# rvp-group/Splat-LOAM

Hardware: AMD Instinct MI355X
Metric: fwd+bwd Msplats/s (higher is better)
Workload: dtype f32; 1 GPU; 500000 surfels, 64x2048 spherical, 1 keyframe/GPU per iteration drawn from a window of 8 keyframes as Mapper.optimize does (sample_geometric, p=0.4): render fwd + mapper loss + bwd + fused Adam (one native sls_mapping_step per iteration); step=one bench step = 10 mapping iterations (1013 steps = 10130 timed iterations), N=500000, H=64, W=2048, keyframes=8, parallelism=keyframe-dp1, status_read=lagged-1, gradient_sums=float atomics

## Files before the change

splat_loam_amd/csrc/sls_sort.hip:

```cpp
#include <cstdlib>
#include "sls_common.hpp"
#include "sls_resort.hpp"
#include "sls_launch.hpp"

namespace sls {

#ifndef SLS_SORT_ROUNDS
#define SLS_SORT_ROUNDS 16
#endif
#ifndef SLS_SORT_WAVES
#define SLS_SORT_WAVES 8
#endif
constexpr int kSortRounds = SLS_SORT_ROUNDS;
constexpr int kSortWaveItems = kWave * kSortRounds;
constexpr int kSortMaxBins = 2048;
constexpr int kDepthKeyBits = 29;

__device__ __forceinline__ uint32_t load_count(const uint32_t *count_ptr, uint32_t cap)
{
    const uint32_t c = *count_ptr;
    return c < cap ? c : cap;
}

__device__ __forceinline__ void resort_verify(int nwin, const uint64_t *__restrict__ edges, uint32_t *__restrict__ flag);
// ... 390 lines not shown

template <typename KeyT, int BITS>
static int tile_sort_emit_chunks(const KeyT *kin, const uint32_t *vin, KeyT *kout, uint32_t *vout,
                                 const uint32_t *chunk_start, uint32_t cap, int shift, uint32_t *cnt, uint32_t *totals,
                                 int nchunks, uint2 *ranges_out, int nranges, uint32_t packed_val_mask, hipStream_t st,
                                 const BlockMaskArgs &bm)
{
    {
        ScopedTimer tm(T_SORT_ROWSCAN, st);
        hipLaunchKernelGGL(sort_rowscan_kernel, dim3(1 << BITS), dim3(256), 0, st, cnt, (const uint32_t *)nullptr, cap, nchunks,
                           totals, nchunks);
    }
    SLS_LAUNCH_CHECK("sort_rowscan_kernel");
    {
        ScopedTimer tm(T_SORT_SCATTER, st);
        const int nblocks = (nchunks + SortBlock<BITS>::kWaves - 1) / SortBlock<BITS>::kWaves;
        hipLaunchKernelGGL((sort_scatter_chunks_kernel<KeyT, BITS>), dim3(nblocks), dim3(64 * SortBlock<BITS>::kWaves), 0, st,
                           kin, vin, kout, vout, chunk_start, cap, shift, (const uint32_t *)cnt, (const uint32_t *)totals,
                           nchunks, ranges_out, nranges, packed_val_mask, bm);
    }
    SLS_LAUNCH_CHECK("sort_scatter_chunks_kernel");
    return SLS_OK;
}

static size_t sort_core_bytes(uint64_t cap)
{
    const uint64_t nchunks = (cap + kSortWaveItems - 1) / kSortWaveItems;
    return (size_t)(kSortMaxBins * (nchunks ? nchunks : 1) + kSortMaxBins) * sizeof(uint32_t);
}
size_t sort_scratch_bytes(uint64_t cap)
{
    return sort_core_bytes(cap) + 2 * sizeof(uint64_t) * (size_t)cap + 64;
}
uint2 *sort_bmask_buffer(void *scratch, uint64_t cap)
{
    return (uint2 *)((char *)scratch + ((sort_core_bytes(cap) + 15) & ~(size_t)15));
}
uint64_t *sort_wide_buffer(void *scratch, uint64_t cap)
{
    return (uint64_t *)(sort_bmask_buffer(scratch, cap) + cap);
}

static void sort_plan(int nbits, int &npasses, int &bits)
{
    npasses = (nbits + 10) / 11;
    bits = (nbits + npasses - 1) / npasses;
    if (bits < 8) bits = 8;
}
int sort_passes(int nbits)
{
    int np, b;
    sort_plan(nbits, np, b);
    return np;
}

template <typename KeyT, int BITS>
static int radix_pass(const KeyT *kin, const uint32_t *vin, KeyT *kout, uint32_t *vout, const uint32_t *count_ptr,
                      uint32_t cap, int shift, uint32_t *cnt, uint32_t *totals, int nchunks, int ,
                      uint2 *ranges_out, int nranges, uint32_t packed_val_mask, hipStream_t st,
                      const BlockMaskArgs &bm)
{
    const int nblocks = (nchunks + SortBlock<BITS>::kWaves - 1) / SortBlock<BITS>::kWaves;
    {
        ScopedTimer tm(T_SORT_HIST, st);
        hipLaunchKernelGGL((sort_hist_kernel<KeyT, BITS>), dim3(nblocks), dim3(64 * SortBlock<BITS>::kWaves), 0, st, kin,
                           count_ptr, cap, shift, cnt, nchunks);
    }
    SLS_LAUNCH_CHECK("sort_hist_kernel");
    {
        ScopedTimer tm(T_SORT_ROWSCAN, st);
        hipLaunchKernelGGL(sort_rowscan_kernel, dim3(1 << BITS), dim3(256), 0, st, cnt, count_ptr, cap, nchunks, totals, 0);
    }
    SLS_LAUNCH_CHECK("sort_rowscan_kernel");
    {
        ScopedTimer tm(T_SORT_SCATTER, st);
        hipLaunchKernelGGL((sort_scatter_kernel<KeyT, BITS>), dim3(nblocks), dim3(64 * SortBlock<BITS>::kWaves), 0, st, kin, vin, kout, vout,
                           count_ptr, cap, shift, (const uint32_t *)cnt, (const uint32_t *)totals, nchunks, ranges_out,
                           nranges, packed_val_mask, bm);
    }
    SLS_LAUNCH_CHECK("sort_scatter_kernel");
    return SLS_OK;
}

template <typename KeyT>
static int radix_sort_pairs_t(KeyT *keys, uint32_t *vals, KeyT *keys_tmp, uint32_t *vals_tmp,
                              const uint32_t *count_ptr, uint32_t cap, int nbits, void *scratch,
                              size_t scratch_bytes, int *result_in_tmp, hipStream_t st,
                              uint2 *ranges_out = nullptr, int nranges = 0, bool drop_sorted_keys = false,
                              int base_shift = 0, BlockMaskArgs bm = BlockMaskArgs{ nullptr, 1, 1.0f, 1 })
{
    *result_in_tmp = 0;
    if (cap == 0 || nbits <= 0) return SLS_OK;
    if (scratch_bytes < sort_scratch_bytes(cap)) {
        set_error("sort scratch too small: %zu < %zu", scratch_bytes, sort_scratch_bytes(cap));
        return SLS_E_SCRATCH;
    }
    const int nchunks = (int)(((uint64_t)cap + kSortWaveItems - 1) / kSortWaveItems);
    uint32_t *cnt = (uint32_t *)scratch;
    int npasses, bits;
    sort_plan(nbits, npasses, bits);
    if (ranges_out && npasses != 1) {
        set_error("internal: ranges need a single-pass sort");
        return SLS_E_ARG;
    }
    uint32_t *totals = cnt + ((size_t)1 << bits) * nchunks;
    KeyT *kb[2] = { keys, keys_tmp };
    uint32_t *vb[2] = { vals, vals_tmp };
    for (int p = 0; p < npasses; ++p) {
        const int shift = base_shift + bits * p;
        const int src = p & 1, dst = src ^ 1;
        const uint32_t packed_val_mask = (vals == nullptr && base_shift > 0) ? ((1u << base_shift) - 1u) : 0u;
        int rc;
        KeyT *kout = (drop_sorted_keys && p + 1 == npasses) ? nullptr : kb[dst];
#define SLS_PASS(B) radix_pass<KeyT, B>(kb[src], vb[src], kout, vb[dst], count_ptr, cap, shift, cnt, totals, nchunks, \
                                        0, ranges_out, nranges, packed_val_mask, st,                           \
                                        (npasses == 1 ? bm : BlockMaskArgs{ nullptr, 1, 1.0f, 1 }))
        switch (bits) {
        case 8: rc = SLS_PASS(8); break;
        case 9: rc = SLS_PASS(9); break;
        case 10: rc = SLS_PASS(10); break;
        default: rc = SLS_PASS(11); break;
        }
#undef SLS_PASS
        if (rc) return rc;
    }
    *result_in_tmp = npasses & 1;
    return SLS_OK;
}

int radix_sort_pairs_u32(uint32_t *keys, uint32_t *vals, uint32_t *keys_tmp, uint32_t *vals_tmp,
                         const uint32_t *count_ptr, uint32_t cap, int nbits, void *scratch, size_t scratch_bytes,
                         int *result_in_tmp, hipStream_t st)
{
    return radix_sort_pairs_t<uint32_t>(keys, vals, keys_tmp, vals_tmp, count_ptr, cap, nbits, scratch,
                                        scratch_bytes, result_in_tmp, st);
}

int radix_sort_pairs_u64(uint64_t *keys, uint32_t *vals, uint64_t *keys_tmp, uint32_t *vals_tmp,
                         const uint32_t *count_ptr, uint32_t cap, int nbits, void *scratch, size_t scratch_bytes,
                         int *result_in_tmp, hipStream_t st)
{
    return radix_sort_pairs_t<uint64_t>(keys, vals, keys_tmp, vals_tmp, count_ptr, cap, nbits, scratch,
                                        scratch_bytes, result_in_tmp, st);
}

__global__ __launch_bounds__(kResortThreads) void resort_sort_kernel(int N, const uint32_t *__restrict__ prev_order,
                                                                     const uint32_t *__restrict__ keys_by_surfel,
                                                                     uint64_t *__restrict__ comp)
{
    __shared__ __attribute__((aligned(16))) ulonglong2 s_pairs[kResortThreads];
    resort_sort_window((int)blockIdx.x, N, prev_order, [&](uint32_t g) { return keys_by_surfel[g]; }, comp, s_pairs);
}

template <bool DIRECT, bool PRE>
__global__ __launch_bounds__(kResortThreads) void resort_merge_kernel(int N, const uint64_t *__restrict__ comp,
                                                                      uint32_t *__restrict__ order,
                                                                      uint64_t *__restrict__ edges,
                                                                      const uint32_t *__restrict__ tiles,
                                                                      uint32_t *__restrict__ block_sums, int GX,
                                                                      const uint2 *__restrict__ erec_box, DirectBin db,
                                                                      uint64_t *comp_out)
{
    static_assert(kResortWindow == 1024 && kResortThreads == 512, "a 256-block of positions = two waves of pairs");
    __shared__ __attribute__((aligned(16))) ulonglong2 s_pairs[kResortThreads];
    __shared__ uint32_t s_part[4][2];
    __shared__ uint32_t s_hist[DIRECT ? kDirectMaxBins : 1];
    __shared__ int s_diff[DIRECT ? kDirectMaxBins + 64 : 1];
    __shared__ int s_wide;
    __shared__ uint64_t s_win[PRE ? 2 * kResortWindow : 1];
    const bool use_diff = DIRECT && GX % 64 == 0 && db.bins % GX == 0 && db.bins / GX <= 64;
    if (DIRECT) {
        for (int d = threadIdx.x; d < db.bins; d += kResortThreads) s_hist[d] = 0u;
        for (int d = threadIdx.x; d < kDirectMaxBins + 64; d += kResortThreads) s_diff[d] = 0;
        if (threadIdx.x == 0) s_wide = 0;
    }
    const int base = blockIdx.x * kResortWindow - kResortWindow / 2, o0 = 2 * (int)threadIdx.x;
    uint64_t e[2];
    if (PRE) {
        uint64_t f[2][2];
#pragma unroll
        for (int a = 0; a < 2; ++a) {
            const int abase = ((int)blockIdx.x - 1 + a) * kResortWindow;
#pragma unroll
            for (int q = 0; q < 2; ++q) {
                const int pos = abase + bitonic_src(o0 + q);
                const uint64_t c = comp[min(max(pos, 0), N - 1)];
                f[a][q] = pos < 0 ? 0ull : (pos < N ? c : ~0ull);
            }
        }
#pragma unroll
        for (int a = 0; a < 2; ++a) {
            bitonic_pairs<kResortWindow>(f[a][0], f[a][1], s_pairs);
            s_win[a * kResortWindow + o0] = f[a][0];
            s_win[a * kResortWindow + o0 + 1] = f[a][1];
        }
        __syncthreads();
#pragma unroll
        for (int q = 0; q < 2; ++q) {
            const int o = bitonic_src(o0 + q);
            e[q] = o < kResortWindow / 2 ? s_win[kResortWindow / 2 + o] : s_win[kResortWindow + o - kResortWindow / 2];
        }
    } else {
#pragma unroll
        for (int q = 0; q < 2; ++q) {
            const int pos = base + bitonic_src(o0 + q);
            const uint64_t c = comp[min(max(pos, 0), N - 1)];
            e[q] = pos < 0 ? 0ull : (pos < N ? c : ~0ull);
        }
    }
    bitonic_pairs<kResortWindow>(e[0], e[1], s_pairs);
    if (comp_out) {
#pragma unroll
        for (int q = 0; q < 2; ++q) {
            const int pos = base + o0 + q;
            if (pos >= 0 && pos < N) comp_out[pos] = e[q];
        }
    }
    uint32_t v = 0;
    if (DIRECT) {
        uint2 er[2];
#pragma unroll
        for (int q = 0; q < 2; ++q) {
            const int pos = base + o0 + q;
            const bool real = pos >= 0 && pos < N;
            const uint32_t g = real ? (uint32_t)e[q] : 0u;
            er[q] = erec_box[g];
            if (!real) er[q].x = 0u;
            if (real) order[pos] = g;
        }
#pragma unroll
        for (int q = 0; q < 2; ++q) {
            const int pos = base + o0 + q;
            if (pos >= 0 && pos < N) db.serec[pos] = er[q];
            if (use_diff) count_rect_rows_diff(er[q].x, GX, s_hist, s_diff, &s_wide);
            else count_rect_tiles_wave(er[q].x, GX, s_hist);
        }
    } else {
#pragma unroll
        for (int q = 0; q < 2; ++q) {
            const int pos = base + o0 + q;
            const bool real = pos >= 0 && pos < N;
            const uint32_t g = real ? (uint32_t)e[q] : 0u;
            const uint32_t tv = tiles[g];
            v += real ? tv : 0u;
            if (real) order[pos] = g;
        }
#pragma unroll
        for (int off = 32; off > 0; off >>= 1) v += __shfl_down(v, off, 64);
        if ((threadIdx.x & 63) == 0) s_part[threadIdx.x >> 7][(threadIdx.x >> 6) & 1] = v;
    }
    const int lo = base < 0 ? -base : 0, hi = min(kResortWindow, N - base) - 1;
#pragma unroll
    for (int q = 0; q < 2; ++q) {
        if (o0 + q == lo) edges[2 * blockIdx.x + 0] = e[q];
        if (o0 + q == hi) edges[2 * blockIdx.x + 1] = e[q];
    }
    __syncthreads();
    if (DIRECT && use_diff && s_wide) {
        diff_finish(GX, db.bins, s_hist, s_diff, (int)threadIdx.x, kResortThreads);
        __syncthreads();
    }
    if (DIRECT) {
        for (int d = threadIdx.x; d < db.bins; d += kResortThreads) {
            const uint32_t c = s_hist[d];
            db.cnt[(size_t)d * db.stride + blockIdx.x] = c;
            if (db.coarse && c) atomicAdd(&db.coarse[(size_t)(blockIdx.x / kDirectGroup) * db.bins + d], c);
        }
    } else if (threadIdx.x < 4) {
        const int blk = (base + (int)threadIdx.x * 256) / 256;
        if (base + (int)threadIdx.x * 256 >= 0 && blk * 256 < N)
            block_sums[blk] = s_part[threadIdx.x][0] + s_part[threadIdx.x][1];
    }
}

__global__ __launch_bounds__(kDirectChunk) void gather_count_kernel(int N, int GX, const uint32_t *__restrict__ order,
                                                                    const uint2 *__restrict__ erec_box,
                                                                    const int4 *__restrict__ rect,
                                                                    const uint32_t *__restrict__ sbox, DirectBin db)
{
    __shared__ uint32_t s_hist[kDirectMaxBins];
    __shared__ int s_diff[kDirectMaxBins + 64];
    __shared__ int s_wide;
    const bool use_diff = GX % 64 == 0 && db.bins % GX == 0 && db.bins / GX <= 64;
    if ((int)threadIdx.x < db.bins) s_hist[threadIdx.x] = 0u;
    for (int d = threadIdx.x; d < kDirectMaxBins + 64; d += kDirectChunk) s_diff[d] = 0;
    if (threadIdx.x == 0) s_wide = 0;
    __syncthreads();
    const int pos = blockIdx.x * kDirectChunk + (int)threadIdx.x;
    uint2 er = make_uint2(0u, 0u);
    if (pos < N) {
        er = load_emit_record(erec_box, rect, sbox, order[pos]);
        if (db.serec) db.serec[pos] = er;
    }
    if (use_diff) count_rect_rows_diff(er.x, GX, s_hist, s_diff, &s_wide);
    else count_rect_tiles_wave(er.x, GX, s_hist);
    __syncthreads();
    if (use_diff && s_wide) {
        diff_finish(GX, db.bins, s_hist, s_diff, (int)threadIdx.x, kDirectChunk);
        __syncthreads();
    }
    if ((int)threadIdx.x < db.bins) {
        const uint32_t c = s_hist[threadIdx.x];
        db.cnt[(size_t)threadIdx.x * db.stride + blockIdx.x] = c;
        if (db.coarse && c) atomicAdd(&db.coarse[(size_t)(blockIdx.x / kDirectGroup) * db.bins + threadIdx.x], c);
    }
}

__device__ __forceinline__ void resort_verify(int nwin, const uint64_t *__restrict__ edges, uint32_t *__restrict__ flag)
{
    for (int b = threadIdx.x; b + 1 < nwin; b += 256)
        if (edges[2 * b + 1] >= edges[2 * (b + 1)]) atomicOr(flag, kResortFailed);
}

__device__ __forceinline__ uint32_t wave_max_scan(uint32_t v)
{
#define SLS_MAXDPP(ctrl_, rows_) v = max(v, (uint32_t)__builtin_amdgcn_update_dpp((int)v, (int)v, ctrl_, rows_, 0xF, false))
    SLS_MAXDPP(0x111, 0xF);
    SLS_MAXDPP(0x112, 0xF);
    SLS_MAXDPP(0x114, 0xF);
    SLS_MAXDPP(0x118, 0xF);
    SLS_MAXDPP(0x142, 0xA);
    SLS_MAXDPP(0x143, 0xC);
#undef SLS_MAXDPP
    return v;
}

constexpr uint32_t kHeavyWave = 1536;
constexpr int kHeavyParts = 4, kHeavyChunks = 16;
template <int BITS, bool PAIRS, int SPLIT>
__global__ __launch_bounds__(kDirectChunk / SPLIT) void bin_direct_kernel(int N, int GX, DirectBin db,
                                                                  const uint32_t *__restrict__ order,
                                                                  const uint2 *__restrict__ erec_box,
                                                                  const int4 *__restrict__ rect,
                                                                  const uint32_t *__restrict__ sbox, uint32_t cap,
                                                                  uint32_t *__restrict__ vals_out, BlockMaskArgs bm,
                                                                  uint2 *__restrict__ ranges_out, int nranges,
                                                                  uint32_t *__restrict__ total_out,
                                                                  uint32_t *__restrict__ overflow, int resort_windows,
                                                                  const uint64_t *__restrict__ resort_edges,
                                                                  uint32_t *__restrict__ fail_flag,
                                                                  uint32_t *__restrict__ status_mirror)
{
    constexpr int BINS = 1 << BITS, TPB = kDirectChunk / SPLIT, WAVES = TPB / 64;
    constexpr int PER = BINS > TPB ? BINS / TPB : 1;
    static_assert(BINS <= kDirectMaxBins && TPB % 64 == 0 && (BINS % TPB == 0 || BINS < TPB), "tiles dealt evenly to the threads");
    __shared__ uint32_t s_cur[WAVES * BINS];
    __shared__ uint32_t s_pre[BINS];
    __shared__ uint4 s_lane[WAVES][64];
    __shared__ uint32_t s_mark[WAVES][64];
    __shared__ uint32_t s_part[WAVES];
    __shared__ uint32_t s_ws[WAVES];
    const int tid = threadIdx.x, lane = tid & 63, w = tid >> 6;
    const int nhelp = SPLIT == 1 ? min(kHeavyChunks, db.nchunks) * (kHeavyParts - 1) : 0;
    const bool helper = (int)blockIdx.x < nhelp;
    const int chunk = helper ? (int)blockIdx.x / (kHeavyParts - 1) : ((int)blockIdx.x - nhelp) / SPLIT;
    const int sub = helper ? 0 : ((int)blockIdx.x - nhelp) % SPLIT;
    const int part = helper ? 1 + (int)blockIdx.x % (kHeavyParts - 1) : 0;
    const bool lead = !helper && chunk == 0 && sub == 0;
    if (resort_windows > 0 && lead) {
        for (int b = tid; b + 1 < resort_windows; b += TPB)
            if (resort_edges[2 * b + 1] >= resort_edges[2 * (b + 1)]) atomicOr(fail_flag, kResortFailed);
    }
    const int pos0 = db.pos0 + chunk * kDirectChunk;
    const int pos = pos0 + sub * TPB + tid;
    const bool real = pos >= 0 && pos < N;
    uint2 er = make_uint2(0u, 0u);
    uint32_t g = 0u;
    if (real) {
        g = order[pos];
// ... 359 lines not shown
        mask = (tile_mask && (uint32_t)(rc.y * rc.w) <= 64u) ? tile_mask[g] : ~0ull;
    }
    const uint64_t box_hi = wide ? ((uint64_t)sbox[g] << 32) : 0ull;
    const uint32_t nrect = (uint32_t)(rc.y * rc.w);
    if (nrect > 64u) mask = ~0ull;
    const uint32_t t = (i < N) ? (nrect <= 64u ? (uint32_t)__popcll(mask & (nrect >= 64u ? ~0ull : ((1ull << nrect) - 1ull))) : nrect) : 0u;
    uint32_t end;
    if (fused.block_sums) {
        __shared__ uint32_t s_wave[EW];
        __shared__ uint32_t s_pre[EW];
        if (fused.resort_windows > 0 && blockIdx.x == 0) resort_verify(fused.resort_windows, fused.resort_edges, fail_flag);
        const int lane = threadIdx.x & 63, wave = threadIdx.x >> 6;
        uint32_t pre = 0;
        for (int b = threadIdx.x; b < (int)blockIdx.x * (EB / 256); b += EB) pre += fused.block_sums[b];
#pragma unroll
        for (int off = 32; off > 0; off >>= 1) pre += __shfl_xor(pre, off, 64);
        uint32_t incl = t;
#pragma unroll
        for (int off = 1; off < 64; off <<= 1) {
            const uint32_t u = __shfl_up(incl, off, 64);
            if (lane >= off) incl += u;
        }
        if (lane == 63) s_wave[wave] = incl;
        if (lane == 0) s_pre[wave] = pre;
        __syncthreads();
        uint32_t wave_prefix = 0;
        for (int w = 0; w < wave; ++w) wave_prefix += s_wave[w];
        uint32_t block_prefix = 0;
#pragma unroll
        for (int w = 0; w < EW; ++w) block_prefix += s_pre[w];
        end = block_prefix + wave_prefix + incl;
        if (blockIdx.x == gridDim.x - 1 && threadIdx.x == EB - 1) *total_out = end;
    } else {
        end = (i < N) ? offsets[i] : 0u;
    }
    if (chunk_start && threadIdx.x == 0) {
        chunk_start[blockIdx.x] = end - t;
        if (blockIdx.x == gridDim.x - 1 && !fused.block_sums) chunk_start[gridDim.x] = offsets[N - 1];
    }
    if (chunk_start && fused.block_sums && blockIdx.x == gridDim.x - 1 && threadIdx.x == EB - 1) chunk_start[gridDim.x] = end;
    bool emit = i < N && t != 0u;
    uint32_t off = end - t;
    if (emit && end > cap) {
        if (overflow) atomicOr(overflow, 1u);
        if (off >= cap) emit = false;
    }
    if (emit) {
        uint32_t bit = 0;
        for (int y = 0; y < rc.w; ++y) {
            const uint32_t row = (uint32_t)(rc.z + y) * (uint32_t)GX;
            for (int k = 0; k < rc.y; ++k, ++bit) {
                if (bit < 64u && !((mask >> bit) & 1ull)) continue;
                int tx = rc.x + k;
                if (tx >= GX) tx -= GX;
                if (off < cap) {
                    const uint32_t tile = row + (uint32_t)tx;
                    if (wide) wide[off] = box_hi | (uint64_t)((tile << pack_shift) | g);
                    else if (vals) { tkeys[off] = tile; vals[off] = g; }
                    else tkeys[off] = (tile << pack_shift) | g;
                    if (hist_cnt) atomicAdd(&s_hist[tile], 1u);
                }
                ++off;
            }
        }
    }
    if (hist_cnt) {
        __syncthreads();
        for (int d = threadIdx.x; d < hist_bins; d += EB) hist_cnt[(size_t)d * gridDim.x + blockIdx.x] = s_hist[d];
    }
}

__global__ __launch_bounds__(256) void tile_ranges_kernel(const uint32_t *__restrict__ tkeys,
                                                          const uint32_t *__restrict__ vals,
                                                          const uint32_t *__restrict__ count_ptr, uint32_t cap,
                                                          const float *__restrict__ depth, uint2 *__restrict__ ranges,
                                                          uint64_t *__restrict__ keys64)
{
    const uint32_t R = load_count(count_ptr, cap);
    const uint32_t j = blockIdx.x * 256 + threadIdx.x;
    if (j >= R) return;
    const uint32_t t = tkeys[j];
    if (j == 0 || tkeys[j - 1] != t) ranges[t].x = j;
    if (j + 1 == R || tkeys[j + 1] != t) ranges[t].y = j + 1;
    if (keys64) keys64[j] = ((uint64_t)t << 32) | (uint64_t)__float_as_uint(depth[vals[j]]);
}

static int bits_for(uint32_t max_value)
{
    int b = 0;
    while (b < 32 && (max_value >> b) != 0) ++b;
    return b;
}

size_t order_scratch_bytes(int N)
{
    const size_t n = (size_t)(N > 0 ? N : 1);
    return sizeof(uint32_t) * (3 * n + (n + 255) / 256 + 64) + sort_scratch_bytes(n) + 16 + n / 32 + 128;
}

struct OrderScratch {
    uint32_t *keys, *keys_tmp, *vals_tmp, *block_sums, *n_dev;
    void *sort_scratch;
    uint64_t *comp;
    bool odd;
    OrderScratch(int N, void *scratch)
    {
        keys = (uint32_t *)scratch; keys_tmp = keys + N; vals_tmp = keys_tmp + N;
        block_sums = vals_tmp + N + 2;
        n_dev = block_sums + (N + 255) / 256;
        sort_scratch = (void *)(n_dev + 32);
        comp = (uint64_t *)(((uintptr_t)keys_tmp + 7) & ~(uintptr_t)7);
        odd = (sort_passes(kDepthKeyBits) & 1) != 0;
    }
};

void depth_order_key_buffers(int N, void *scratch, uint32_t *order, uint32_t **keys, uint32_t **vals0, uint32_t **n_dev)
{
    const OrderScratch s(N, scratch);
    *keys = s.keys;
    *vals0 = s.odd ? s.vals_tmp : order;
    *n_dev = s.n_dev;
}

uint64_t *resort_comp_buffer(int N, void *scratch) { return OrderScratch(N, scratch).comp; }

int launch_depth_order_scan(const DepthOrderScan &a, hipStream_t st, ScanHandoff *handoff)
{
    const int N = a.N, reuse_order = a.reuse_order;
    uint32_t *order = a.order;
    const DirectBin *direct = a.direct;
    if (a.scratch_bytes < order_scratch_bytes(N)) {
        set_error("depth-order scratch too small: %zu < %zu", a.scratch_bytes, order_scratch_bytes(N));
        return SLS_E_SCRATCH;
    }
    const int nb = (N + 255) / 256;
    const OrderScratch s(N, a.scratch);
    uint32_t *keys = s.keys, *block_sums = s.block_sums;
    uint32_t *v0 = s.odd ? s.vals_tmp : order, *v1 = s.odd ? order : s.vals_tmp;
    int resort_windows = 0;
    const uint64_t *resort_edges = nullptr;
    if (reuse_order && a.fail_flag) {
        uint64_t *comp = s.comp;
        uint64_t *edges = (uint64_t *)(((uintptr_t)s.sort_scratch + 7) & ~(uintptr_t)7);
        const int nA = (N + kResortWindow - 1) / kResortWindow;
        const int nB = (N + kResortWindow / 2 + kResortWindow - 1) / kResortWindow;
        ScopedTimer tm(T_RESORT, st);
        if (!a.window_sort_done) {
            hipLaunchKernelGGL(resort_sort_kernel, dim3(nA), dim3(kResortThreads), 0, st, N, (const uint32_t *)order,
                               (const uint32_t *)keys, comp);
            SLS_LAUNCH_CHECK("resort_sort_kernel");
        }
        const DirectBin no_db = { nullptr, nullptr, nullptr, 0, 0, 0 };
        const bool count_here = direct != nullptr && handoff != nullptr;
        uint64_t *comp2 = edges + 2 * (size_t)nB + 2;
#define SLS_MERGE(PRE_, last_, in_, out_)                                                                                    \
        do {                                                                                                                 \
            if (count_here && (last_))                                                                                       \
                hipLaunchKernelGGL((resort_merge_kernel<true, PRE_>), dim3(nB), dim3(kResortThreads), 0, st, N,               \
                                   (const uint64_t *)(in_), order, edges, a.tiles, block_sums, a.GX, (const uint2 *)a.erec_box,      \
                                   *direct, (uint64_t *)(out_));                                                              \
            else                                                                                                             \
                hipLaunchKernelGGL((resort_merge_kernel<false, PRE_>), dim3(nB), dim3(kResortThreads), 0, st, N,              \
                                   (const uint64_t *)(in_), order, edges, a.tiles, block_sums, a.GX, (const uint2 *)a.erec_box,      \
                                   no_db, (uint64_t *)(out_));                                                                \
        } while (0)
        SLS_MERGE(false, reuse_order <= 1, comp, reuse_order > 1 ? comp : nullptr);
        SLS_LAUNCH_CHECK("resort_merge_kernel");
        uint64_t *cin = comp, *cout = comp2;
        for (int round = 1; round < reuse_order; ++round) {
            const bool last = round + 1 == reuse_order;
            SLS_MERGE(true, last, cin, last ? nullptr : cout);
            SLS_LAUNCH_CHECK("resort_merge_kernel (further round)");
            uint64_t *t = cin; cin = cout; cout = t;
        }
#undef SLS_MERGE
        if (count_here) {
            if (direct->nchunks != nB || direct->pos0 != -kResortWindow / 2) {
                set_error("internal: the direct binning's chunks are not the repair's windows");
                return SLS_E_ARG;
            }
            handoff->counted = 1;
        }
        resort_windows = nB;
        resort_edges = edges;
    } else {
        int which = 0;
        int rc = radix_sort_pairs_t<uint32_t>(keys, v0, s.keys_tmp, v1, s.n_dev, (uint32_t)N, kDepthKeyBits, s.sort_scratch,
                                              sort_scratch_bytes((uint64_t)N), &which, st, nullptr, 0, true);
        if (rc) return rc;
        if ((which != 0) != s.odd) {
            set_error("internal: depth order ended in the wrong buffer");
            return SLS_E_ARG;
        }
    }
    if (handoff && direct && resort_windows == 0) {
        *handoff = ScanHandoff{ nullptr, 0, nullptr, 0 };
        return SLS_OK;
    }
    if (handoff && resort_windows > 0) {
        *handoff = ScanHandoff{ block_sums, resort_windows, resort_edges, handoff->counted };
        return SLS_OK;
    }
    ScopedTimer tm(T_SCAN, st);
    if (resort_windows == 0) {
        hipLaunchKernelGGL(gather_block_sums_kernel, dim3(nb), dim3(256), 0, st, N, (const uint32_t *)order, a.tiles,
                           block_sums);
        SLS_LAUNCH_CHECK("gather_block_sums_kernel");
    }
    if (handoff) {
        *handoff = ScanHandoff{ block_sums, 0, nullptr, handoff->counted };
        return SLS_OK;
    }
    hipLaunchKernelGGL(gather_scan_final_kernel, dim3(nb), dim3(256), 0, st, N, (const uint32_t *)order, a.tiles,
                       (const uint32_t *)block_sums, a.offsets, a.total_out, resort_windows, resort_edges, a.fail_flag);
    SLS_LAUNCH_CHECK("gather_scan_final_kernel");
    return SLS_OK;
}

int launch_bin_sort(const DevCam &cam, const BinSortLaunch &a, hipStream_t st, int *sorted_in_tmp, const uint2 **bmask_out)
{
    const int T = cam.GX * cam.GY, N = a.N;
    const uint32_t cap = a.cap;
    void *scratch = a.scratch;
    uint32_t *ranges = a.ranges, *tkeys = a.tkeys, *vals = a.vals, *tkeys_tmp = a.tkeys_tmp, *vals_tmp = a.vals_tmp;
    *sorted_in_tmp = 0;
    if (bmask_out) *bmask_out = nullptr;
    if (cap == 0 || N == 0) {
        SLS_HIP_CHECK(hipMemsetAsync(ranges, 0, sizeof(uint32_t) * 2 * (size_t)T, st));
        return SLS_OK;
    }
    if (a.scratch_bytes < sort_scratch_bytes(cap)) {
        set_error("sort scratch too small: %zu < %zu", a.scratch_bytes, sort_scratch_bytes(cap));
        return SLS_E_SCRATCH;
    }
    const int tile_bits = bits_for((uint32_t)(T - 1));
    const bool fused_ranges = sort_passes(tile_bits) == 1 && a.keys64_out == nullptr;
    if (!fused_ranges) SLS_HIP_CHECK(hipMemsetAsync(ranges, 0, sizeof(uint32_t) * 2 * (size_t)T, st));
    const int idx_bits = bits_for((uint32_t)(N - 1)) > 0 ? bits_for((uint32_t)(N - 1)) : 1;
    const bool packed = fused_ranges && tile_bits + idx_bits <= 32;
    const int bins = 1 << (tile_bits < 8 ? 8 : tile_bits);
    constexpr int eb = 256;
    const int nemit = (N + eb - 1) / eb;
    uint32_t *cnt = (uint32_t *)scratch, *totals = cnt + (size_t)bins * nemit, *chunk_start = totals + bins;
    const bool emit_hist = fused_ranges && (size_t)bins * nemit <= (size_t)400000 &&
                           ((size_t)bins * nemit + bins + nemit + 1) * sizeof(uint32_t) <= sort_core_bytes(cap);
    const bool long_lists = a.bmask_mode == 1 || (a.bmask_mode == 0 && (uint64_t)cap >= 1500ull * (uint64_t)T);
    BlockMaskArgs bm = { nullptr, cam.GX, 1.0f / (float)cam.GX, (cam.GX * kTileW) / 8 };
    uint64_t *wide = nullptr;
    if (a.sbox && bmask_out && packed && kTileW == 16 && kTileH == 16 && long_lists &&
        block_box_fits(cam.GX * kTileW, cam.H)) {
        bm.out = sort_bmask_buffer(scratch, cap);
        wide = sort_wide_buffer(scratch, cap);
        *bmask_out = bm.out;
    }
    {
        ScopedTimer tm(T_EMIT_KEYS, st);
        hipLaunchKernelGGL(emit_tiles_kernel<eb>, dim3(nemit), dim3(eb), 0, st, N, cam.GX, a.order, (const int4 *)a.rect, a.tiles,
                           a.tile_mask, (const int4 *)a.erec, a.offsets, cap, tkeys, packed ? (uint32_t *)nullptr : vals, a.overflow,
                           packed ? idx_bits : 0, a.handoff ? *a.handoff : ScanHandoff{ nullptr, 0, nullptr, 0 }, a.total_out,
                           a.overflow, emit_hist ? cnt : (uint32_t *)nullptr, bins, emit_hist ? chunk_start : (uint32_t *)nullptr,
                           a.sbox, wide);
    }
    SLS_LAUNCH_CHECK("emit_tiles_kernel");
    int which = 0;
    int rc;
    if (emit_hist) {
        const uint32_t *vin = packed ? nullptr : vals;
        const int shift = packed ? idx_bits : 0;
        const uint32_t pmask = packed ? ((1u << idx_bits) - 1u) : 0u;
#define SLS_CASE(K_, B) case B: rc = tile_sort_emit_chunks<K_, B>(wide ? (const K_ *)wide : (const K_ *)tkeys, vin, (K_ *)nullptr, vals_tmp, chunk_start, \
                                                              cap, shift, cnt, totals, nemit, (uint2 *)ranges, T, pmask, st, bm); break;
        if (wide) {
            switch (tile_bits < 8 ? 8 : tile_bits) { SLS_CASE(uint64_t, 8) SLS_CASE(uint64_t, 9) SLS_CASE(uint64_t, 10) default: SLS_CASE(uint64_t, 11) }
        } else {
            switch (tile_bits < 8 ? 8 : tile_bits) { SLS_CASE(uint32_t, 8) SLS_CASE(uint32_t, 9) SLS_CASE(uint32_t, 10) default: SLS_CASE(uint32_t, 11) }
        }
#undef SLS_CASE
        which = 1;
    } else if (wide) {
        rc = radix_sort_pairs_t<uint64_t>(wide, nullptr, nullptr, vals_tmp, a.count_ptr, cap, tile_bits, scratch,
                                          a.scratch_bytes, &which, st, (uint2 *)ranges, T, true, idx_bits, bm);
    } else if (packed) {
        rc = radix_sort_pairs_t<uint32_t>(tkeys, nullptr, tkeys_tmp, vals_tmp, a.count_ptr, cap, tile_bits, scratch,
                                          a.scratch_bytes, &which, st, (uint2 *)ranges, T, true, idx_bits);
    } else {
        rc = radix_sort_pairs_t<uint32_t>(tkeys, vals, tkeys_tmp, vals_tmp, a.count_ptr, cap, tile_bits, scratch,
                                          a.scratch_bytes, &which, st, fused_ranges ? (uint2 *)ranges : nullptr, T,
                                          fused_ranges);
    }
    if (rc) return rc;
    *sorted_in_tmp = which;
    if (!fused_ranges) {
        ScopedTimer tm(T_TILE_RANGES, st);
        hipLaunchKernelGGL(tile_ranges_kernel, dim3((cap + 255) / 256), dim3(256), 0, st,
                           (const uint32_t *)(which ? tkeys_tmp : tkeys), (const uint32_t *)(which ? vals_tmp : vals),
                           a.count_ptr, cap, a.depth, (uint2 *)ranges, a.keys64_out);
        SLS_LAUNCH_CHECK("tile_ranges_kernel");
    }
    return SLS_OK;
}


static int direct_bins(const DevCam &cam)
{
    const int tb = bits_for((uint32_t)(cam.GX * cam.GY - 1));
    return 1 << (tb < 8 ? 8 : tb);
}
static size_t direct_max_stride(int N)
{
    const size_t nchunks = (size_t)(N + kDirectChunk / 2 + kDirectChunk - 1) / kDirectChunk;
    return (nchunks + kDirectGroup - 1) / kDirectGroup * kDirectGroup;
}
bool bin_direct_possible(const DevCam &cam, int N, uint32_t cap)
{
    if (N <= 0 || cap == 0 || cam.tile_cull != 0 || cam.GX > 512 || cam.GY > 64) return false;
    if (cam.GX * cam.GY > kDirectMaxBins) return false;
    if (!block_box_fits(cam.GX * kTileW, cam.H)) return false;
    const size_t bins = (size_t)direct_bins(cam);
    return (bins * direct_max_stride(N) + bins + direct_coarse_words(cam, N)) * sizeof(uint32_t) <= sort_core_bytes(cap);
}
size_t direct_coarse_words(const DevCam &cam, int N)
{
    const size_t nchunks = (size_t)(N + kDirectChunk / 2 + kDirectChunk - 1) / kDirectChunk;
    return ((nchunks + kDirectGroup - 1) / kDirectGroup) * (size_t)direct_bins(cam);
}
DirectBin make_direct_bin(const DevCam &cam, int N, void *sort_scratch, uint2 *serec, bool repaired, bool coarse)
{
// ... 53 lines not shown
```

Measured before the change: 1865 Msplats/s.

## Fuse multi-round depth-order repair merges into one kernel with on-demand escalation

Replaces the chain of per-round resort merge launches (each writing an intermediate comp buffer) with a single launch. Each block checks whether any window boundary in its dependency cone is out of order. Only in that case does it load a cone of windows into dynamic LDS and run the merge levels locally, skipping windows that are already ordered. This removes extra kernel launches and global round-trips when the order is already nearly sorted, at the cost of large dynamic LDS per block and a cap of 4 rounds.

```diff
diff --git a/splat_loam_amd/csrc/sls_sort.hip b/splat_loam_amd/csrc/sls_sort.hip
--- a/splat_loam_amd/csrc/sls_sort.hip
+++ b/splat_loam_amd/csrc/sls_sort.hip
@@ -566,14 +566,14 @@
     resort_sort_window((int)blockIdx.x, N, prev_order, [&](uint32_t g) { return keys_by_surfel[g]; }, comp, s_pairs);
 }
 
-template <bool DIRECT, bool PRE>
+template <bool DIRECT, bool ESC>
 __global__ __launch_bounds__(kResortThreads) void resort_merge_kernel(int N, const uint64_t *__restrict__ comp,
                                                                       uint32_t *__restrict__ order,
                                                                       uint64_t *__restrict__ edges,
                                                                       const uint32_t *__restrict__ tiles,
                                                                       uint32_t *__restrict__ block_sums, int GX,
                                                                       const uint2 *__restrict__ erec_box, DirectBin db,
-                                                                      uint64_t *comp_out)
+                                                                      int rounds)
 {
     static_assert(kResortWindow == 1024 && kResortThreads == 512, "a 256-block of positions = two waves of pairs");
     __shared__ __attribute__((aligned(16))) ulonglong2 s_pairs[kResortThreads];
@@ -581,7 +581,7 @@
     __shared__ uint32_t s_hist[DIRECT ? kDirectMaxBins : 1];
     __shared__ int s_diff[DIRECT ? kDirectMaxBins + 64 : 1];
     __shared__ int s_wide;
-    __shared__ uint64_t s_win[PRE ? 2 * kResortWindow : 1];
+    __shared__ int s_escalate;
     const bool use_diff = DIRECT && GX % 64 == 0 && db.bins % GX == 0 && db.bins / GX <= 64;
     if (DIRECT) {
         for (int d = threadIdx.x; d < db.bins; d += kResortThreads) s_hist[d] = 0u;
@@ -589,46 +589,57 @@
         if (threadIdx.x == 0) s_wide = 0;
     }
     const int base = blockIdx.x * kResortWindow - kResortWindow / 2, o0 = 2 * (int)threadIdx.x;
+    auto pair_at = [&](int pos) -> uint64_t {
+        const uint64_t c = comp[min(max(pos, 0), N - 1)];
+        return pos < 0 ? 0ull : (pos < N ? c : ~0ull);
+    };
+    bool out_of_order = false;
+    if (ESC && (int)threadIdx.x < 2 * rounds - 2) {
+        const int j = (int)blockIdx.x - (rounds - 1) + (int)threadIdx.x, m = j * kResortWindow + kResortWindow / 2;
+        if (m > 0 && m < N) {
+            const uint64_t l0 = pair_at(m - kResortWindow / 2 - 1), l1 = pair_at(m - 1);
+            const uint64_t r0 = pair_at(m), r1 = pair_at(m + kResortWindow / 2);
+            out_of_order = !(max(l0, l1) < min(r0, r1));
+        }
+    }
     uint64_t e[2];
-    if (PRE) {
-        uint64_t f[2][2];
-#pragma unroll
-        for (int a = 0; a < 2; ++a) {
-            const int abase = ((int)blockIdx.x - 1 + a) * kResortWindow;
-#pragma unroll
-            for (int q = 0; q < 2; ++q) {
-                const int pos = abase + bitonic_src(o0 + q);
-                const uint64_t c = comp[min(max(pos, 0), N - 1)];
-                f[a][q] = pos < 0 ? 0ull : (pos < N ? c : ~0ull);
+#pragma unroll
+    for (int q = 0; q < 2; ++q) e[q] = pair_at(base + bitonic_src(o0 + q));
+    bool escalate = false;
+    if (ESC) {
+        if (threadIdx.x < 64) {
+            const bool any = __ballot(out_of_order) != 0ull;
+            if (threadIdx.x == 0) s_escalate = any ? 1 : 0;
+        }
+        __syncthreads();
+        escalate = s_escalate != 0;
+    }
+    if (ESC && escalate) {
+        extern __shared__ __attribute__((aligned(16))) uint64_t s_cone[];
+        const int nwin = 2 * rounds, cone0 = ((int)blockIdx.x - rounds) * kResortWindow;
+        for (int i = threadIdx.x; i < nwin * kResortWindow; i += kResortThreads) s_cone[i] = pair_at(cone0 + i);
+        __syncthreads();
+        const auto word = [&](int i) -> uint64_t {
+            const uint64_t v = s_cone[i];
+            return ((uint64_t)__builtin_amdgcn_readfirstlane((uint32_t)(v >> 32)) << 32) | __builtin_amdgcn_readfirstlane((uint32_t)v);
+        };
+        for (int level = 1; level < nwin; ++level) {
+            const bool shifted = (level & 1) != 0;
+            const int first = level >> 1, last = nwin - 1 - first - (shifted ? 1 : 0);
+            for (int w = first; w <= last; ++w) {
+                const int off = w * kResortWindow + (shifted ? kResortWindow / 2 : 0);
+                if (word(off + kResortWindow / 2 - 1) <= word(off + kResortWindow / 2)) continue;
+                uint64_t f0 = s_cone[off + bitonic_src(o0)], f1 = s_cone[off + bitonic_src(o0 + 1)];
+                bitonic_pairs<kResortWindow>(f0, f1, s_pairs);
+                s_cone[off + o0] = f0;
+                s_cone[off + o0 + 1] = f1;
+                __syncthreads();
             }
         }
-#pragma unroll
-        for (int a = 0; a < 2; ++a) {
-            bitonic_pairs<kResortWindow>(f[a][0], f[a][1], s_pairs);
-            s_win[a * kResortWindow + o0] = f[a][0];
-            s_win[a * kResortWindow + o0 + 1] = f[a][1];
-        }
-        __syncthreads();
-#pragma unroll
-        for (int q = 0; q < 2; ++q) {
-            const int o = bitonic_src(o0 + q);
-            e[q] = o < kResortWindow / 2 ? s_win[kResortWindow / 2 + o] : s_win[kResortWindow + o - kResortWindow / 2];
-        }
+        e[0] = s_cone[rounds * kResortWindow - kResortWindow / 2 + o0];
+        e[1] = s_cone[rounds * kResortWindow - kResortWindow / 2 + o0 + 1];
     } else {
-#pragma unroll
-        for (int q = 0; q < 2; ++q) {
-            const int pos = base + bitonic_src(o0 + q);
-            const uint64_t c = comp[min(max(pos, 0), N - 1)];
-            e[q] = pos < 0 ? 0ull : (pos < N ? c : ~0ull);
-        }
-    }
-    bitonic_pairs<kResortWindow>(e[0], e[1], s_pairs);
-    if (comp_out) {
-#pragma unroll
-        for (int q = 0; q < 2; ++q) {
-            const int pos = base + o0 + q;
-            if (pos >= 0 && pos < N) comp_out[pos] = e[q];
-        }
+        bitonic_pairs<kResortWindow>(e[0], e[1], s_pairs);
     }
     uint32_t v = 0;
     if (DIRECT) {
@@ -1294,27 +1305,28 @@
         }
         const DirectBin no_db = { nullptr, nullptr, nullptr, 0, 0, 0 };
         const bool count_here = direct != nullptr && handoff != nullptr;
-        uint64_t *comp2 = edges + 2 * (size_t)nB + 2;
-#define SLS_MERGE(PRE_, last_, in_, out_)                                                                                    \
-        do {                                                                                                                 \
-            if (count_here && (last_))                                                                                       \
-                hipLaunchKernelGGL((resort_merge_kernel<true, PRE_>), dim3(nB), dim3(kResortThreads), 0, st, N,               \
-                                   (const uint64_t *)(in_), order, edges, a.tiles, block_sums, a.GX, (const uint2 *)a.erec_box,      \
-                                   *direct, (uint64_t *)(out_));                                                              \
-            else                                                                                                             \
-                hipLaunchKernelGGL((resort_merge_kernel<false, PRE_>), dim3(nB), dim3(kResortThreads), 0, st, N,              \
-                                   (const uint64_t *)(in_), order, edges, a.tiles, block_sums, a.GX, (const uint2 *)a.erec_box,      \
-                                   no_db, (uint64_t *)(out_));                                                                \
-        } while (0)
-        SLS_MERGE(false, reuse_order <= 1, comp, reuse_order > 1 ? comp : nullptr);
+        const int rounds = reuse_order;
+        if (rounds > 4) {
+            set_error("depth-order repair: at most 4 rounds (%d)", rounds);
+            return SLS_E_ARG;
+        }
+        const size_t cone_bytes = rounds > 1 ? (size_t)2 * rounds * kResortWindow * sizeof(uint64_t) : 0;
+        static bool lds_allowed = false;
+        if (rounds > 1 && !lds_allowed) {
+            const int most = 2 * 4 * kResortWindow * (int)sizeof(uint64_t);
+            SLS_HIP_CHECK(hipFuncSetAttribute(reinterpret_cast<const void *>(resort_merge_kernel<true, true>),
+                                              hipFuncAttributeMaxDynamicSharedMemorySize, most));
+            SLS_HIP_CHECK(hipFuncSetAttribute(reinterpret_cast<const void *>(resort_merge_kernel<false, true>),
+                                              hipFuncAttributeMaxDynamicSharedMemorySize, most));
+            lds_allowed = true;
+        }
+#define SLS_MERGE(DIRECT_, ESC_, db_)                                                                                        \
+        hipLaunchKernelGGL((resort_merge_kernel<DIRECT_, ESC_>), dim3(nB), dim3(kResortThreads), cone_bytes, st, N,          \
+                           (const uint64_t *)comp, order, edges, a.tiles, block_sums, a.GX, (const uint2 *)a.erec_box, db_,  \
+                           rounds)
+        if (count_here) { if (rounds > 1) SLS_MERGE(true, true, *direct); else SLS_MERGE(true, false, *direct); }
+        else { if (rounds > 1) SLS_MERGE(false, true, no_db); else SLS_MERGE(false, false, no_db); }
         SLS_LAUNCH_CHECK("resort_merge_kernel");
-        uint64_t *cin = comp, *cout = comp2;
-        for (int round = 1; round < reuse_order; ++round) {
-            const bool last = round + 1 == reuse_order;
-            SLS_MERGE(true, last, cin, last ? nullptr : cout);
-            SLS_LAUNCH_CHECK("resort_merge_kernel (further round)");
-            uint64_t *t = cin; cin = cout; cout = t;
-        }
 #undef SLS_MERGE
         if (count_here) {
             if (direct->nchunks != nB || direct->pos0 != -kResortWindow / 2) {
```

New measurement: 1944 Msplats/s (median of 6 runs). 1.04x the previous value.
